# google-research/rigl

Hardware: NVIDIA H100
Metric: sparse_train_step_images_per_sec_resnet50_erk80 (higher is better)
Workload: dtype bf16

## Files before the change

rigl_b200/csrc/igemm_tc.cu:

```cuda
#include <cuda.h>
#include <cuda_bf16.h>

#include <stdio.h>
#include <stdlib.h>

#include <mutex>

#include "common.cuh"
#include "conv_common.cuh"
#include "tc_ptx.cuh"

namespace rigl {

using namespace ptx;

constexpr int kMaxTaps = 9;
constexpr int kBM = 128;
constexpr int kBK = 64;
constexpr int kThreads = 384;
constexpr int kConsumerWarp0 = 4;
constexpr int kConsumerWarps = 8;
constexpr int kConsumerThreads = 256;

struct TapInfo {
// ... 235 lines not shown
      }
    }
  } else if (warp >= kConsumerWarp0) {
    const int cw = warp - kConsumerWarp0;
    const int wg = cw >> 2;
    const int row = 64 * wg + 16 * (cw & 3) + (lane >> 2);
    const bool issuer = (cw == 0 && lane == 0);
    float acc[BN / 2];
    int stage = 0; uint32_t phase = 0;
    uint32_t slab_ctr = 0;
    uint32_t res_phase = 0;
    float* bn_row = (kEpi == kEpiPlain && p.bn_partial) ? p.bn_partial + (size_t)blockIdx.x * 2 * p.N : nullptr;
    if (bn_row) {
      for (int i = cw * 32 + lane; i < 2 * p.N; i += kConsumerThreads) bn_row[i] = 0.f;
      __threadfence_block();
      named_bar_sync(1, kConsumerThreads);
    }
    int tile_ctr = 0;
    for (int tile = first; tile < total; tile += step, ++tile_ctr) {
      const int n_tile = tile % p.n_tiles;
      const int m_tile = tile / p.n_tiles;
      uint32_t* live = live_cons[wg][tile_ctr & 1];
      if ((cw & 3) == 0) build_live_mask<kBN64>(p, n_tile, lane, live);
      named_bar_sync(3 + wg, 128);
      const bool masked = live_mask_used(p);
      zero_acc(acc);
      int prev = -1;
      const int nkb = p.ntaps * p.kblks;
      for (int j = 0; j < nkb; ++j) {
        if (masked && !((live[j >> 5] >> (j & 31)) & 1u)) continue;
        mbar_wait(full_bar(stage), phase);
        const uint32_t a_src = smem_base + stage * kStageBytes;
        const uint64_t da = make_smem_desc(a_src + (uint32_t)wg * 64u * 128u, 16, 1024);
        const uint64_t db = make_smem_desc(a_src + kABytes, 16, 1024);
        fence_regs(acc);
        wgmma_fence();
#pragma unroll
        for (int k = 0; k < kBK / 16; ++k)
          Wgmma<BN>::template ss<0, 0>(acc, da + 2 * k, db + 2 * k);
        wgmma_commit();
        wgmma_wait<1>();
        if (prev >= 0 && lane == 0) mbar_arrive(empty_bar(prev));
        prev = stage;
        if (++stage == STAGES) { stage = 0; phase ^= 1u; }
      }
      wgmma_wait<0>();
      fence_regs(acc);
      if (prev >= 0 && lane == 0) mbar_arrive(empty_bar(prev));

      const int tw = m_tile % p.tiles_w;
      const int th = (m_tile / p.tiles_w) % p.tiles_h;
      const int tn = m_tile / (p.tiles_w * p.tiles_h);
      bool ok[2]; long long o_pix[2];
#pragma unroll
      for (int h = 0; h < 2; ++h) {
        const int r = row + 8 * h;
        const int pw = tw * p.bw + r % p.bw;
        const int ph = th * p.bh + (r / p.bw) % p.bh;
        const int pn = tn * p.bn + r / (p.bw * p.bh);
        ok[h] = pw < p.GW && ph < p.GH && pn < p.NB;
        o_pix[h] = p.o_off + pn * p.o_sn + ph * p.o_sh + pw * p.o_sw;
      }
      if (kEpi != kEpiPlain || p.tma_store) {
#pragma unroll
        for (int s = 0; s < kBN64; ++s) {
          const int co0 = n_tile * BN + 64 * s;
          if (co0 >= p.N) break;
          const uint32_t slab = out_base + (uint32_t)(slab_ctr & 1) * kSlabBytes;
          if (issuer) tma_store_wait_read<1>();
          named_bar_sync(1, kConsumerThreads);
          if constexpr (kLoadsSlab) {
            if (kEpi == kEpiReluGate || ep.residual) {
              if (issuer) {
                mbar_arrive_expect_tx(res_bar, kSlabBytes);
                tma_load_4d(slab, rmap, res_bar, co0, tw * p.bw, th * p.bh, tn * p.bn);
              }
              mbar_wait(res_bar, res_phase);
              res_phase ^= 1u;
            }
          }
          if constexpr (kBnApply) {
            if (s == 0) stage_slab_bn<0>(acc, slab, row, ok[0], ok[1], lane, ep, co0, p.N);
            else stage_slab_bn<(kBN64 > 1 ? 1 : 0)>(acc, slab, row, ok[0], ok[1], lane, ep, co0, p.N);
          } else if constexpr (kEpi != kEpiPlain) {
            constexpr bool kGate = kEpi == kEpiReluGate;
            if (s == 0) stage_slab_relu<0, kGate>(acc, slab, row, ok[0], ok[1], lane);
            else stage_slab_relu<(kBN64 > 1 ? 1 : 0), kGate>(acc, slab, row, ok[0], ok[1], lane);
          } else {
            if (s == 0) stage_slab<0>(acc, slab, row, ok[0], ok[1], lane);
            else stage_slab<(kBN64 > 1 ? 1 : 0)>(acc, slab, row, ok[0], ok[1], lane);
          }
          fence_proxy_async_smem();
          named_bar_sync(1, kConsumerThreads);
          if (issuer) {
            tma_store_4d(&omap, slab, co0, tw * p.bw, th * p.bh, tn * p.bn);
            tma_store_commit();
          }
          if (bn_row && wg == 0) slab_bn_stats(slab, cw, lane, bn_row, co0, p.N);
          ++slab_ctr;
        }
      } else {
#pragma unroll
        for (int jc = 0; jc < BN / 8; ++jc) {
#pragma unroll
          for (int h = 0; h < 2; ++h) {
#pragma unroll
            for (int e = 0; e < 2; ++e) {
              const int co = n_tile * BN + 8 * jc + 2 * (lane & 3) + e;
              if (ok[h] && co < p.N) {
                float a = acc[4 * jc + 2 * h + e];
                if (p.bias) a += __ldg(p.bias + co);
                if (p.out_bf16) p.out_bf16[o_pix[h] + co] = __float2bfloat16(a);
                if (p.out_f32) p.out_f32[o_pix[h] + co] = a;
              }
            }
          }
        }
      }
    }
    if (p.tma_store && issuer) tma_store_wait_all();
  }
}

template <int BN, int STAGES>
__global__ void __launch_bounds__(kThreads, 1)
k_igemm_kmajor(const __grid_constant__ TMaps4 amaps, const __grid_constant__ CUtensorMap bmap,
               const __grid_constant__ CUtensorMap omap, const IgemmParams p) {
  kmajor_body<BN, STAGES, kEpiPlain>(amaps, bmap, omap, p, nullptr, BnEpilogue{});
}

template <int BN, int STAGES>
__global__ void __launch_bounds__(kThreads, 1)
k_igemm_kmajor_bn(const __grid_constant__ TMaps4 amaps, const __grid_constant__ CUtensorMap bmap,
                  const __grid_constant__ CUtensorMap omap, const IgemmParams p,
                  const __grid_constant__ CUtensorMap rmap, const BnEpilogue ep) {
  kmajor_body<BN, STAGES, kEpiBn>(amaps, bmap, omap, p, &rmap, ep);
}

template <int BN, int STAGES, bool kGate>
__global__ void __launch_bounds__(kThreads, 1)
k_igemm_kmajor_relu(const __grid_constant__ TMaps4 amaps, const __grid_constant__ CUtensorMap bmap,
                    const __grid_constant__ CUtensorMap omap, const IgemmParams p,
                    const __grid_constant__ CUtensorMap rmap) {
  kmajor_body<BN, STAGES, kGate ? kEpiReluGate : kEpiRelu>(amaps, bmap, omap, p, &rmap, BnEpilogue{});
}

struct WgradParams {
  int ntaps;
  TapInfo taps[kMaxTaps];
  int GW, GH, NB;
  int bw, bh, bn;
  int tiles_w, tiles_h, tiles_n;
  int pblocks, splits, pblocks_per_split;
  int ci, co;
  int m_tiles, n_tiles;
  float* out;
  long long split_stride;
};

template <int BN, int STAGES>
__global__ void __launch_bounds__(kThreads, 1)
k_igemm_wgrad(const __grid_constant__ TMaps4 xmaps, const __grid_constant__ CUtensorMap dymap,
              const WgradParams p) {
  extern __shared__ __align__(1024) uint8_t smem_raw[];
  constexpr uint32_t kABytes = kBM * kBK * 2;
  constexpr uint32_t kBBytes = BN * kBK * 2;
  constexpr uint32_t kStageBytes = kABytes + kBBytes;
  constexpr uint32_t kBox = 64 * 64 * 2;
  constexpr int kBBoxes = BN / 64;

  const uint32_t smem_base = (smem_u32(smem_raw) + 1023u) & ~1023u;
  const uint32_t bar_base = smem_base + STAGES * kStageBytes;
  auto full_bar = [&](int s) { return bar_base + 8u * s; };
  auto empty_bar = [&](int s) { return bar_base + 8u * (STAGES + s); };

  const int warp = threadIdx.x >> 5, lane = threadIdx.x & 31;
  if (threadIdx.x == 0) {
    for (int i = 0; i < 4; ++i) prefetch_tmap(&xmaps.a[i]);
    prefetch_tmap(&dymap);
    for (int s = 0; s < STAGES; ++s) { mbar_init(full_bar(s), 1); mbar_init(empty_bar(s), kConsumerWarps); }
    fence_barrier_init();
  }
  __syncthreads();

  const int mcount = p.ntaps * p.m_tiles;
  const int units_per_split = mcount * p.n_tiles;
  const int total_units = units_per_split * p.splits;
  const int first = blockIdx.x, step = gridDim.x;

  if (warp == 0) {
    int stage = 0; uint32_t phase = 0;
    for (int q = first; q < total_units; q += step) {
      const int split = q / units_per_split;
      const int r = q % units_per_split;
      const int n_tile = r % p.n_tiles;
      const int mi = r / p.n_tiles;
      const bool live = mi < mcount;
      const TapInfo tap = p.taps[live ? mi / p.m_tiles : 0];
      const int c_base = live ? (mi % p.m_tiles) * kBM : (1 << 28);
      const int pb0 = split * p.pblocks_per_split;
      const int pb1 = min(pb0 + p.pblocks_per_split, p.pblocks);
      int tw = pb0 % p.tiles_w, th = (pb0 / p.tiles_w) % p.tiles_h, tn = pb0 / (p.tiles_w * p.tiles_h);
      for (int pb = pb0; pb < pb1; ++pb) {
        mbar_wait(empty_bar(stage), phase ^ 1u);
        if (elect_one()) {
          const uint32_t a_dst = smem_base + stage * kStageBytes;
          const uint32_t b_dst = a_dst + kABytes;
          mbar_arrive_expect_tx(full_bar(stage), kStageBytes);
#pragma unroll
          for (int h = 0; h < kBM / 64; ++h)
            tma_load_4d(a_dst + h * kBox, &xmaps.a[tap.map_id], full_bar(stage), c_base + h * 64,
                        tw * p.bw + tap.dw, th * p.bh + tap.dh, tn * p.bn);
#pragma unroll
          for (int h = 0; h < kBBoxes; ++h)
            tma_load_4d(b_dst + h * kBox, &dymap, full_bar(stage), n_tile * BN + h * 64, tw * p.bw,
                        th * p.bh, tn * p.bn);
        }
        __syncwarp();
        if (++tw == p.tiles_w) { tw = 0; if (++th == p.tiles_h) { th = 0; ++tn; } }
        if (++stage == STAGES) { stage = 0; phase ^= 1u; }
      }
    }
  } else if (warp >= kConsumerWarp0) {
    const int cw = warp - kConsumerWarp0;
    const int wg = cw >> 2;
    const int row = 64 * wg + 16 * (cw & 3) + (lane >> 2);
    float acc[BN / 2];
    int stage = 0; uint32_t phase = 0;
    for (int q = first; q < total_units; q += step) {
      const int split = q / units_per_split;
      const int r = q % units_per_split;
      const int n_tile = r % p.n_tiles;
      const int mi = r / p.n_tiles;
      const bool live = mi < mcount;
      const int tap_idx = live ? mi / p.m_tiles : 0;
      const int pb0 = split * p.pblocks_per_split;
      const int pb1 = min(pb0 + p.pblocks_per_split, p.pblocks);
      zero_acc(acc);
      int prev = -1;
      for (int pb = pb0; pb < pb1; ++pb) {
        mbar_wait(full_bar(stage), phase);
        const uint32_t a_src = smem_base + stage * kStageBytes;
        const uint64_t da = make_smem_desc(a_src + (uint32_t)wg * kBox, kBox, 1024);
        const uint64_t db = make_smem_desc(a_src + kABytes, kBox, 1024);
        fence_regs(acc);
        wgmma_fence();
#pragma unroll
        for (int k = 0; k < kBK / 16; ++k)
          Wgmma<BN>::template ss<1, 1>(acc, da + 128 * k, db + 128 * k);
        wgmma_commit();
        wgmma_wait<1>();
        if (prev >= 0 && lane == 0) mbar_arrive(empty_bar(prev));
        prev = stage;
        if (++stage == STAGES) { stage = 0; phase ^= 1u; }
      }
      wgmma_wait<0>();
      fence_regs(acc);
      if (prev >= 0 && lane == 0) mbar_arrive(empty_bar(prev));

      const int m0 = live ? (mi % p.m_tiles) * kBM : p.ci;
      float* base = p.out + (long long)split * p.split_stride + (long long)p.taps[tap_idx].b_tap * p.ci * p.co;
#pragma unroll
      for (int h = 0; h < 2; ++h) {
        const int ci = m0 + row + 8 * h;
        if (ci >= p.ci) continue;
#pragma unroll
        for (int jc = 0; jc < BN / 8; ++jc) {
          const int co = n_tile * BN + 8 * jc + 2 * (lane & 3);
          if (co < p.co)
            *reinterpret_cast<float2*>(base + (long long)ci * p.co + co) =
                make_float2(acc[4 * jc + 2 * h], acc[4 * jc + 2 * h + 1]);
        }
      }
    }
  }
}

__global__ void k_splitk_reduce(const float* __restrict__ part, long long split_stride, int splits,
                                float* __restrict__ dw, long long n, float beta) {
  const long long i = ((long long)blockIdx.x * blockDim.x + threadIdx.x) * 4;
  if (i >= n) return;
  if (i + 3 < n) {
    float4 acc = beta != 0.f ? *reinterpret_cast<const float4*>(dw + i) : make_float4(0.f, 0.f, 0.f, 0.f);
    for (int s = 0; s < splits; ++s) {
      const float4 v = *reinterpret_cast<const float4*>(part + (long long)s * split_stride + i);
      acc.x += v.x; acc.y += v.y; acc.z += v.z; acc.w += v.w;
    }
    *reinterpret_cast<float4*>(dw + i) = acc;
  } else {
    for (long long j = i; j < n; ++j) {
      float a = beta != 0.f ? dw[j] : 0.f;
      for (int s = 0; s < splits; ++s) a += part[(long long)s * split_stride + j];
      dw[j] = a;
    }
  }
}

typedef CUresult (*EncodeTiledFn)(CUtensorMap*, CUtensorMapDataType, cuuint32_t, void*, const cuuint64_t*,
                                  const cuuint64_t*, const cuuint32_t*, const cuuint32_t*, CUtensorMapInterleave,
                                  CUtensorMapSwizzle, CUtensorMapL2promotion, CUtensorMapFloatOOBfill);

static EncodeTiledFn g_encode = nullptr;
static bool g_bn_stats_always = false;
static bool g_halo = true;
static int g_num_sms = 0;
static std::once_flag g_once;
static int g_init_status = RIGL_OK;

static void init_driver() {
  void* fn = nullptr;
  cudaDriverEntryPointQueryResult qres;
  cudaError_t e = cudaGetDriverEntryPoint("cuTensorMapEncodeTiled", &fn, cudaEnableDefault, &qres);
  if (e != cudaSuccess || fn == nullptr || qres != cudaDriverEntryPointSuccess) {
    set_error("cuTensorMapEncodeTiled not available from the driver (%s)", cudaGetErrorString(e));
    g_init_status = RIGL_ERR_DRIVER;
    return;
  }
  g_encode = reinterpret_cast<EncodeTiledFn>(fn);
  if (const char* e = getenv("RIGL_HALO3X3")) g_halo = !(e[0] == '0');
  int dev = 0;
  cudaGetDevice(&dev);
  cudaDeviceGetAttribute(&g_num_sms, cudaDevAttrMultiProcessorCount, dev);
  if (g_num_sms <= 0) g_num_sms = kNumSmsHint;
}

static int ensure_driver() {
  static thread_local bool ctx_ready = false;
  if (!ctx_ready) {
    cudaFree(0);
    ctx_ready = true;
  }
  std::call_once(g_once, init_driver);
  return g_init_status;
}

static int make_tmap_swz(CUtensorMap* out, const void* base, int rank, const uint64_t* dims,
                         const uint64_t* strides_bytes , const uint32_t* box, CUtensorMapSwizzle swz) {
  cuuint32_t estr[5] = {1, 1, 1, 1, 1};
  cuuint64_t gdim[5], gstr[4];
  cuuint32_t bx[5];
  for (int i = 0; i < rank; ++i) { gdim[i] = dims[i]; bx[i] = box[i]; }
  for (int i = 0; i + 1 < rank; ++i) gstr[i] = strides_bytes[i];
  CUresult r = g_encode(out, CU_TENSOR_MAP_DATA_TYPE_BFLOAT16, (cuuint32_t)rank, const_cast<void*>(base), gdim,
                        gstr, bx, estr, CU_TENSOR_MAP_INTERLEAVE_NONE, swz,
                        CU_TENSOR_MAP_L2_PROMOTION_L2_128B, CU_TENSOR_MAP_FLOAT_OOB_FILL_NONE);
  if (r != CUDA_SUCCESS) {
    set_error("cuTensorMapEncodeTiled failed (%d): rank %d dims [%llu,%llu,%llu,%llu] box [%u,%u,%u,%u]", (int)r,
              rank, (unsigned long long)dims[0], (unsigned long long)(rank > 1 ? dims[1] : 0),
              (unsigned long long)(rank > 2 ? dims[2] : 0), (unsigned long long)(rank > 3 ? dims[3] : 0), box[0],
              rank > 1 ? box[1] : 0, rank > 2 ? box[2] : 0, rank > 3 ? box[3] : 0);
    return RIGL_ERR_DRIVER;
  }
  return RIGL_OK;
}
static int make_tmap(CUtensorMap* out, const void* base, int rank, const uint64_t* dims,
                     const uint64_t* strides_bytes , const uint32_t* box) {
  return make_tmap_swz(out, base, rank, dims, strides_bytes, box, CU_TENSOR_MAP_SWIZZLE_128B);
}

static int make_act_map(CUtensorMap* out, const void* base, int nb, int h, int w, int c, int pitch, int s, int rh,
                        int rw, const uint32_t box[4]) {
  const uint64_t hr = (h - rh + s - 1) / s, wr = (w - rw + s - 1) / s;
  const uint64_t dims[4] = {(uint64_t)c, wr, hr, (uint64_t)nb};
  const uint64_t strides[3] = {(uint64_t)s * pitch * 2, (uint64_t)s * w * pitch * 2, (uint64_t)h * w * pitch * 2};
  const uint8_t* p = static_cast<const uint8_t*>(base) + ((size_t)rh * w + rw) * pitch * 2;
  return make_tmap(out, p, 4, dims, strides, box);
}

static void choose_box(int gw, int gh, int nb, int total, int* bw, int* bh, int* bn) {
  long long best = -1;
  for (int w = 1; w <= total; w *= 2)
    for (int h = 1; w * h <= total; h *= 2) {
      const int n = total / (w * h);
      const long long padded = (long long)((gw + w - 1) / w * w) * ((gh + h - 1) / h * h) * ((nb + n - 1) / n * n);
      const long long score = padded * 1024 - w * 16 - h;
      if (best < 0 || score < best) { best = score; *bw = w; *bh = h; *bn = n; }
    }
}

static inline int floordiv(int a, int b) { return (a >= 0) ? a / b : -((-a + b - 1) / b); }
static inline int posmod(int a, int b) { return ((a % b) + b) % b; }

template <typename P>
static void set_pixel_tiling(P& p, int gw, int gh, int nb, int box_pixels) {
  p.GW = gw; p.GH = gh; p.NB = nb;
  choose_box(gw, gh, nb, box_pixels, &p.bw, &p.bh, &p.bn);
  p.tiles_w = (gw + p.bw - 1) / p.bw; p.tiles_h = (gh + p.bh - 1) / p.bh; p.tiles_n = (nb + p.bn - 1) / p.bn;
}

template <typename P>
static int set_conv_taps(P& p, TMaps4* maps, const ConvGeom& g, const void* x, const uint32_t box[4]) {
  bool made[4] = {false, false, false, false};
  p.ntaps = 0;
  for (int kh = 0; kh < g.ksize; ++kh)
    for (int kw = 0; kw < g.ksize; ++kw) {
      const int rh = posmod(kh - g.pad, g.stride), rw = posmod(kw - g.pad, g.stride);
      const int id = rh * g.stride + rw;
      if (!made[id]) {
        const int rc = make_act_map(&maps->a[id], x, g.batch, g.in_h, g.in_w, g.cin, g.x_pitch, g.stride, rh, rw, box);
        if (rc != RIGL_OK) return rc;
        made[id] = true;
      }
      TapInfo& t = p.taps[p.ntaps++];
      t.map_id = (int8_t)id; t.dh = (int8_t)floordiv(kh - g.pad, g.stride); t.dw = (int8_t)floordiv(kw - g.pad, g.stride);
      t.b_tap = kh * g.ksize + kw;
    }
  for (int i = 0; i < 4; ++i) if (!made[i]) maps->a[i] = maps->a[p.taps[0].map_id];
  return RIGL_OK;
}

int tc_max_ctas() {
  ensure_driver();
  return g_num_sms > 0 ? g_num_sms : kNumSmsHint;
}

bool tc_supported(const ConvGeom& g, int which) {
  if (g.x_pitch % 8 || g.cout % 8) return false;
  if (which == 1 && g.cin % 8) return false;
  if (g.stride != 1 && g.stride != 2) return false;
  if (g.ksize * g.ksize > kMaxTaps) return false;
  (void)which;
  return true;
}

// ... 98 lines not shown
  int rc = ensure_driver();
  if (rc != RIGL_OK) return rc;
  const PackedLayout L = packed_layout(g.taps(), g.cin, g.cout);
  const uint8_t* pk = static_cast<const uint8_t*>(packed);
  {
    HaloParams hp = {};
    if (y != nullptr && y_f32 == nullptr && bias == nullptr && halo_fprop_ok(g, &hp)) {
      if (relu)
        return halo_launch_kmajor(hp, x, g.cin, g.x_pitch, pk + L.off_fprop, L.cin_pad, g.cout, y, g.cout, false, s,
                                  true);
      if (bn_apply != nullptr) {
        set_error("fused BN apply: layer runs on the halo kernels");
        return RIGL_ERR_UNSUPPORTED;
      }
      if (bn_partial != nullptr) {
        set_error("fused BN statistics: layer runs on the halo kernels");
        return RIGL_ERR_UNSUPPORTED;
      }
      return halo_launch_kmajor(hp, x, g.cin, g.x_pitch, pk + L.off_fprop, L.cin_pad, g.cout, y, g.cout, false, s);
    }
  }
  if (bn_partial != nullptr && !g_bn_stats_always) {
    const int K = g.taps() * g.cin;
    if (!(K >= 512 || (K >= 256 && g.cout <= 128))) {
      set_error("fused BN statistics: not profitable for this shape (K = %d, cout = %d)", K, g.cout);
      return RIGL_ERR_UNSUPPORTED;
    }
  }
  IgemmParams p = {};
  set_pixel_tiling(p, g.out_w, g.out_h, g.batch, 128);
  p.kblks = (g.cin + kBK - 1) / kBK;
  p.N = g.cout;
  p.out_bf16 = static_cast<__nv_bfloat16*>(y); p.out_f32 = y_f32; p.bias = bias;
  p.o_off = 0; p.o_sw = g.cout; p.o_sh = (long long)g.out_w * g.cout; p.o_sn = (long long)g.out_h * g.out_w * g.cout;
  p.nnz = reinterpret_cast<const uint32_t*>(pk + L.off_nnz);
  p.nnz_tap_stride = L.n_tiles * L.k_tiles; p.nnz_n_stride = L.k_tiles; p.nnz_k_stride = 1;
  p.bn_partial = bn_partial;
  TMaps4 amaps;
  const uint32_t abox[4] = {(uint32_t)kBK, (uint32_t)p.bw, (uint32_t)p.bh, (uint32_t)p.bn};
  rc = set_conv_taps(p, &amaps, g, x, abox);
  if (rc != RIGL_OK) return rc;
  const int bn_tile = pick_bn(g.cout);
  CUtensorMap bmap;
  const uint64_t bdims[3] = {(uint64_t)L.cin_pad, (uint64_t)g.cout, (uint64_t)g.taps()};
  const uint64_t bstr[2] = {(uint64_t)L.cin_pad * 2, (uint64_t)g.cout * L.cin_pad * 2};
  const uint32_t bbox[3] = {(uint32_t)kBK, (uint32_t)bn_tile, 1};
  rc = make_tmap(&bmap, pk + L.off_fprop, 3, bdims, bstr, bbox);
  if (rc != RIGL_OK) return rc;
  CUtensorMap omap = bmap;
  p.tma_store = (y != nullptr && y_f32 == nullptr && bias == nullptr) ? 1 : 0;
  if (p.tma_store) {
    rc = make_act_map(&omap, y, g.batch, g.out_h, g.out_w, g.cout, g.cout, 1, 0, 0, abox);
    if (rc != RIGL_OK) return rc;
  }
  if (bn_partial) {
    p.bn_partial = bn_partial;
    p.n_tiles = (g.cout + bn_tile - 1) / bn_tile;
    if (bn_rows) *bn_rows = kmajor_grid(p);
  }
  if (bn_apply) {
    CUtensorMap rmap = omap;
    if (bn_apply->residual) {
      rc = make_act_map(&rmap, bn_apply->residual, g.batch, g.out_h, g.out_w, g.cout, g.cout, 1, 0, 0, abox);
      if (rc != RIGL_OK) return rc;
    }
    const BnEpilogue ep = {bn_apply->scale, bn_apply->shift, bn_apply->relu ? 1 : 0, bn_apply->residual ? 1 : 0};
    return dispatch_kmajor(g.cout, amaps, bmap, omap, p, bn_tile, s, &rmap, &ep);
  }
  if (relu) return dispatch_kmajor(g.cout, amaps, bmap, omap, p, bn_tile, s, nullptr, nullptr, kReluFprop);
  return dispatch_kmajor(g.cout, amaps, bmap, omap, p, bn_tile, s);
}

int tc_dgrad(const ConvGeom& g, const void* dy, const void* packed, void* dx, void* ws, size_t ws_bytes,
             cudaStream_t s, const void* gate) {
  (void)ws; (void)ws_bytes;
  int rc = ensure_driver();
  if (rc != RIGL_OK) return rc;
  const PackedLayout L = packed_layout(g.taps(), g.cin, g.cout);
  const uint8_t* pk = static_cast<const uint8_t*>(packed);
  const int st = g.stride;
  {
    HaloParams hp = {};
    if (halo_dgrad_ok(g, &hp)) {
      if (gate != nullptr) {
        set_error("gated dgrad: layer runs on the halo kernels");
        return RIGL_ERR_UNSUPPORTED;
      }
      return halo_launch_kmajor(hp, dy, g.cout, g.cout, pk + L.off_dgrad, L.cout_pad, g.cin, dx, g.x_pitch, true, s);
    }
  }
  if (gate != nullptr && st != 1) {
    set_error("gated dgrad: only the single-launch stride-1 dgrad has the gate");
    return RIGL_ERR_UNSUPPORTED;
  }
  bool need_zero = false;
  for (int ph = 0; ph < st && !need_zero; ++ph)
    for (int pw = 0; pw < st; ++pw) {
      int n = 0;
      for (int kh = 0; kh < g.ksize; ++kh)
        for (int kw = 0; kw < g.ksize; ++kw)
          if (posmod(ph + g.pad - kh, st) == 0 && posmod(pw + g.pad - kw, st) == 0) ++n;
      if (n == 0) need_zero = true;
    }
  if (need_zero) RIGL_CUDA(cudaMemsetAsync(dx, 0, (size_t)g.in_pixels() * g.x_pitch * 2, s));
  for (int ph = 0; ph < st; ++ph)
    for (int pw = 0; pw < st; ++pw) {
      IgemmParams p = {};
      const int gh = (g.in_h - ph + st - 1) / st, gw = (g.in_w - pw + st - 1) / st;
      if (gh <= 0 || gw <= 0) continue;
      p.ntaps = 0;
      for (int kh = 0; kh < g.ksize; ++kh)
        for (int kw = 0; kw < g.ksize; ++kw)
          if (posmod(ph + g.pad - kh, st) == 0 && posmod(pw + g.pad - kw, st) == 0) {
            TapInfo& t = p.taps[p.ntaps++];
            t.map_id = 0; t.dh = (int8_t)((ph + g.pad - kh) / st); t.dw = (int8_t)((pw + g.pad - kw) / st);
            t.b_tap = kh * g.ksize + kw;
          }
      if (p.ntaps == 0) continue;
      set_pixel_tiling(p, gw, gh, g.batch, 128);
      p.kblks = (g.cout + kBK - 1) / kBK;
      p.N = g.cin;
      p.nnz = reinterpret_cast<const uint32_t*>(pk + L.off_nnz);
      p.nnz_tap_stride = L.n_tiles * L.k_tiles; p.nnz_n_stride = 1; p.nnz_k_stride = L.k_tiles;
      TMaps4 amaps;
      const uint32_t abox[4] = {(uint32_t)kBK, (uint32_t)p.bw, (uint32_t)p.bh, (uint32_t)p.bn};
      rc = make_act_map(&amaps.a[0], dy, g.batch, g.out_h, g.out_w, g.cout, g.cout, 1, 0, 0, abox);
      if (rc != RIGL_OK) return rc;
      for (int i = 1; i < 4; ++i) amaps.a[i] = amaps.a[0];
      const int bn_tile = pick_bn(g.cin);
      CUtensorMap bmap;
      const uint64_t bdims[3] = {(uint64_t)L.cout_pad, (uint64_t)g.cin, (uint64_t)g.taps()};
      const uint64_t bstr[2] = {(uint64_t)L.cout_pad * 2, (uint64_t)g.cin * L.cout_pad * 2};
      const uint32_t bbox[3] = {(uint32_t)kBK, (uint32_t)bn_tile, 1};
      rc = make_tmap(&bmap, pk + L.off_dgrad, 3, bdims, bstr, bbox);
      if (rc != RIGL_OK) return rc;
      CUtensorMap omap;
      rc = make_act_map(&omap, dx, g.batch, g.in_h, g.in_w, g.cin, g.x_pitch, st, ph, pw, abox);
      if (rc != RIGL_OK) return rc;
      p.tma_store = 1;
      if (gate != nullptr) {
        CUtensorMap xmap;
        rc = make_act_map(&xmap, gate, g.batch, g.in_h, g.in_w, g.cin, g.x_pitch, st, ph, pw, abox);
        if (rc != RIGL_OK) return rc;
        rc = dispatch_kmajor(g.cin, amaps, bmap, omap, p, bn_tile, s, &xmap, nullptr, kReluGateDgrad);
        if (rc != RIGL_OK) return rc;
        continue;
      }
      rc = dispatch_kmajor(g.cin, amaps, bmap, omap, p, bn_tile, s);
      if (rc != RIGL_OK) return rc;
    }
  return RIGL_OK;
}

template <int BN, int STAGES>
static int launch_wgrad(const TMaps4& xmaps, const CUtensorMap& dymap, const WgradParams& p, cudaStream_t s) {
  constexpr size_t smem = (size_t)STAGES * (kBM * kBK * 2 + BN * kBK * 2) + 1024 + 256;
  static_assert(smem <= 227 * 1024, "wgrad kernel exceeds the shared memory of an SM");
  static bool configured = false;
  if (!configured) {
    RIGL_CUDA(cudaFuncSetAttribute(k_igemm_wgrad<BN, STAGES>, cudaFuncAttributeMaxDynamicSharedMemorySize, (int)smem));
    configured = true;
  }
  const int units = p.ntaps * p.m_tiles * p.n_tiles * p.splits;
  const int grid = units < g_num_sms ? units : g_num_sms;
  k_igemm_wgrad<BN, STAGES><<<grid, kThreads, smem, s>>>(xmaps, dymap, p);
  RIGL_LAUNCH_CHECK("k_igemm_wgrad");
  return RIGL_OK;
}

int tc_wgrad(const ConvGeom& g, const void* x, const void* dy, float* dw, float beta, void* ws, size_t ws_bytes,
             cudaStream_t s) {
  int rc = ensure_driver();
  if (rc != RIGL_OK) return rc;
  {
    HaloParams hp = {};
    if (halo_wgrad_ok(g, &hp)) {
      const size_t need = halo_wgrad_ws_elems(g, hp) * sizeof(float);
      float* wsf = reinterpret_cast<float*>((reinterpret_cast<uintptr_t>(ws) + 255) & ~(uintptr_t)255);
      if (ws == nullptr || ws_bytes < need + 256) {
        set_error("rigl_conv2d_wgrad_dense: workspace %zu < required %zu", ws_bytes, need + 256);
        return RIGL_ERR_WORKSPACE;
      }
      rc = halo_launch_wgrad(hp, g, x, dy, wsf, s);
      if (rc != RIGL_OK) return rc;
      const long long n_w9 = (long long)9 * g.cin * g.cout;
      const long long threads = (n_w9 + 3) / 4;
      k_splitk_reduce<<<(unsigned)((threads + 255) / 256), 256, 0, s>>>(wsf, n_w9, halo_wgrad_grid(hp), dw, n_w9, beta);
      RIGL_LAUNCH_CHECK("k_splitk_reduce");
      return RIGL_OK;
    }
  }
  WgradParams p = {};
  set_pixel_tiling(p, g.out_w, g.out_h, g.batch, 64);
  p.pblocks = p.tiles_w * p.tiles_h * p.tiles_n;
  const int bn_tile = wgrad_bn_tile(g);
  const size_t elems = wgrad_ws_elems(g, &p.splits, &p.pblocks_per_split, p.bw, p.bh, p.bn, bn_tile);
  p.ci = g.cin; p.co = g.cout;
  p.m_tiles = (g.cin + kBM - 1) / kBM; p.n_tiles = (g.cout + bn_tile - 1) / bn_tile;
  const long long n_w = (long long)g.taps() * g.cin * g.cout;
  const bool direct = (p.splits == 1 && beta == 0.f);
  if (!direct) {
    const size_t need = elems * sizeof(float);
    if (ws == nullptr || ws_bytes < need + 256) {
      set_error("rigl_conv2d_wgrad_dense: workspace %zu < required %zu", ws_bytes, need + 256);
      return RIGL_ERR_WORKSPACE;
    }
    p.out = reinterpret_cast<float*>((reinterpret_cast<uintptr_t>(ws) + 255) & ~(uintptr_t)255);
    p.split_stride = n_w;
  } else {
    p.out = dw; p.split_stride = 0;
  }
  TMaps4 xmaps;
  const uint32_t box[4] = {64, (uint32_t)p.bw, (uint32_t)p.bh, (uint32_t)p.bn};
  rc = set_conv_taps(p, &xmaps, g, x, box);
  if (rc != RIGL_OK) return rc;
  CUtensorMap dymap;
  rc = make_act_map(&dymap, dy, g.batch, g.out_h, g.out_w, g.cout, g.cout, 1, 0, 0, box);
  if (rc != RIGL_OK) return rc;
  rc = (bn_tile == 128) ? launch_wgrad<128, 6>(xmaps, dymap, p, s) : launch_wgrad<64, 8>(xmaps, dymap, p, s);
  if (rc != RIGL_OK) return rc;
  if (!direct) {
    const long long threads = (n_w + 3) / 4;
    k_splitk_reduce<<<(unsigned)((threads + 255) / 256), 256, 0, s>>>(p.out, p.split_stride, p.splits, dw, n_w, beta);
    RIGL_LAUNCH_CHECK("k_splitk_reduce");
  }
  return RIGL_OK;
}

}
```

rigl_b200/csrc/tc_ptx.cuh:

```cuda
#pragma once
#include <cuda.h>
#include <cuda_runtime.h>
#include <stdint.h>

namespace rigl {
namespace ptx {

__device__ __forceinline__ uint32_t smem_u32(const void* p) {
  return static_cast<uint32_t>(__cvta_generic_to_shared(p));
}

__device__ __forceinline__ bool elect_one() {
  uint32_t pred;
  asm volatile(
      "{\n"
      ".reg .pred p;\n"
      "elect.sync _|p, 0xffffffff;\n"
      "selp.u32 %0, 1, 0, p;\n"
      "}\n"
      : "=r"(pred));
  return pred != 0;
}

__device__ __forceinline__ void mbar_init(uint32_t bar, uint32_t count) {
  asm volatile("mbarrier.init.shared::cta.b64 [%0], %1;" ::"r"(bar), "r"(count) : "memory");
}
__device__ __forceinline__ void fence_barrier_init() {
  asm volatile("fence.mbarrier_init.release.cluster;" ::: "memory");
}
__device__ __forceinline__ void mbar_arrive_expect_tx(uint32_t bar, uint32_t bytes) {
  asm volatile("mbarrier.arrive.expect_tx.shared::cta.b64 _, [%0], %1;" ::"r"(bar), "r"(bytes) : "memory");
}
__device__ __forceinline__ void mbar_arrive(uint32_t bar) {
  asm volatile("mbarrier.arrive.shared::cta.b64 _, [%0];" ::"r"(bar) : "memory");
}
__device__ __forceinline__ void mbar_wait(uint32_t bar, uint32_t parity) {
  uint32_t done;
  uint32_t spins = 0;
  long long t0 = 0;
  do {
    asm volatile(
        "{\n"
        ".reg .pred p;\n"
        "mbarrier.try_wait.parity.shared::cta.b64 p, [%1], %2;\n"
        "selp.u32 %0, 1, 0, p;\n"
        "}\n"
        : "=r"(done)
        : "r"(bar), "r"(parity)
        : "memory");
    if (!done && (++spins & 0xFFFu) == 0) {
      const long long now = clock64();
      if (t0 == 0) t0 = now;
      else if (now - t0 > 8000000000ll) __trap();
    }
  } while (!done);
}

__device__ __forceinline__ void prefetch_tmap(const CUtensorMap* m) {
  asm volatile("prefetch.tensormap [%0];" ::"l"(reinterpret_cast<uint64_t>(m)) : "memory");
}
__device__ __forceinline__ void tma_load_4d(uint32_t dst, const CUtensorMap* m, uint32_t bar, int c0, int c1,
                                            int c2, int c3) {
  asm volatile(
      "cp.async.bulk.tensor.4d.shared::cluster.global.mbarrier::complete_tx::bytes [%0], [%1, {%3, %4, %5, %6}], [%2];"
      ::"r"(dst), "l"(reinterpret_cast<uint64_t>(m)), "r"(bar), "r"(c0), "r"(c1), "r"(c2), "r"(c3)
      : "memory");
}
__device__ __forceinline__ void tma_load_3d(uint32_t dst, const CUtensorMap* m, uint32_t bar, int c0, int c1,
                                            int c2) {
  asm volatile(
      "cp.async.bulk.tensor.3d.shared::cluster.global.mbarrier::complete_tx::bytes [%0], [%1, {%3, %4, %5}], [%2];"
      ::"r"(dst), "l"(reinterpret_cast<uint64_t>(m)), "r"(bar), "r"(c0), "r"(c1), "r"(c2)
      : "memory");
}

__device__ __forceinline__ void tma_store_4d(const CUtensorMap* m, uint32_t src, int c0, int c1, int c2, int c3) {
  asm volatile("cp.async.bulk.tensor.4d.global.shared::cta.bulk_group [%0, {%2, %3, %4, %5}], [%1];" ::"l"(
                   reinterpret_cast<uint64_t>(m)),
               "r"(src), "r"(c0), "r"(c1), "r"(c2), "r"(c3)
               : "memory");
}
__device__ __forceinline__ void tma_store_commit() { asm volatile("cp.async.bulk.commit_group;" ::: "memory"); }
template <int N>
__device__ __forceinline__ void tma_store_wait_read() {
  asm volatile("cp.async.bulk.wait_group.read %0;" ::"n"(N) : "memory");
}
__device__ __forceinline__ void tma_store_wait_all() { asm volatile("cp.async.bulk.wait_group 0;" ::: "memory"); }
__device__ __forceinline__ void fence_proxy_async_smem() { asm volatile("fence.proxy.async.shared::cta;" ::: "memory"); }
__device__ __forceinline__ void named_bar_sync(int id, int nthreads) {
  asm volatile("bar.sync %0, %1;" ::"r"(id), "r"(nthreads) : "memory");
}

__device__ __forceinline__ void wgmma_fence() { asm volatile("wgmma.fence.sync.aligned;" ::: "memory"); }
__device__ __forceinline__ void wgmma_commit() { asm volatile("wgmma.commit_group.sync.aligned;" ::: "memory"); }
template <int N>
__device__ __forceinline__ void wgmma_wait() {
  asm volatile("wgmma.wait_group.sync.aligned %0;" ::"n"(N) : "memory");
}
template <int R>
__device__ __forceinline__ void fence_regs(float (&d)[R]) {
#pragma unroll
  for (int i = 0; i < R; ++i) asm volatile("" : "+f"(d[i])::"memory");
}

constexpr uint32_t kSwz128 = 1, kSwz32 = 3;
__device__ __forceinline__ uint64_t make_smem_desc(uint32_t saddr, uint32_t lbo_bytes, uint32_t sbo_bytes,
                                                   uint32_t swz = kSwz128) {
  uint64_t d = 0;
  d |= (uint64_t)((saddr >> 4) & 0x3FFFu);
  d |= (uint64_t)((lbo_bytes >> 4) & 0x3FFFu) << 16;
  d |= (uint64_t)((sbo_bytes >> 4) & 0x3FFFu) << 32;
  d |= (uint64_t)swz << 62;
  return d;
}

__device__ __forceinline__ void ldmatrix_x4(uint32_t (&r)[4], uint32_t addr) {
  asm volatile("ldmatrix.sync.aligned.m8n8.x4.shared.b16 {%0, %1, %2, %3}, [%4];"
               : "=r"(r[0]), "=r"(r[1]), "=r"(r[2]), "=r"(r[3]) : "r"(addr) : "memory");
}
__device__ __forceinline__ void ldmatrix_x4_trans(uint32_t (&r)[4], uint32_t addr) {
  asm volatile("ldmatrix.sync.aligned.m8n8.x4.trans.shared.b16 {%0, %1, %2, %3}, [%4];"
               : "=r"(r[0]), "=r"(r[1]), "=r"(r[2]), "=r"(r[3]) : "r"(addr) : "memory");
}
__device__ __forceinline__ uint32_t swz128(uint32_t addr) { return addr ^ (((addr >> 7) & 7u) << 4); }
__device__ __forceinline__ uint32_t swz32(uint32_t addr) { return addr ^ (((addr >> 7) & 1u) << 4); }

template <int N> struct Wgmma;
template <> struct Wgmma<64> {
  template <int TA, int TB>
  static __device__ __forceinline__ void ss(float (&d)[32], uint64_t da, uint64_t db) {
    asm volatile(
        "{\n.reg .pred p;\nsetp.ne.b32 p, 1, 0;\nwgmma.mma_async.sync.aligned.m64n64k16.f32.bf16.bf16 "
        "{%0, %1, %2, %3, %4, %5, %6, %7, %8, %9, %10, %11, %12, %13, %14, %15, %16, %17, %18, %19, %20, %21, %22, %23, %24, %25, %26, %27, %28, %29, %30, %31}, %32, %33, p, 1, 1, %34, %35;\n}\n"
        : "+f"(d[0]), "+f"(d[1]), "+f"(d[2]), "+f"(d[3]), "+f"(d[4]), "+f"(d[5]), "+f"(d[6]), "+f"(d[7]), "+f"(d[8]), "+f"(d[9]), "+f"(d[10]), "+f"(d[11]), "+f"(d[12]), "+f"(d[13]), "+f"(d[14]), "+f"(d[15]), "+f"(d[16]), "+f"(d[17]), "+f"(d[18]), "+f"(d[19]), "+f"(d[20]), "+f"(d[21]), "+f"(d[22]), "+f"(d[23]), "+f"(d[24]), "+f"(d[25]), "+f"(d[26]), "+f"(d[27]), "+f"(d[28]), "+f"(d[29]), "+f"(d[30]), "+f"(d[31])
        : "l"(da), "l"(db), "n"(TA), "n"(TB));
  }
  template <int TB>
  static __device__ __forceinline__ void rs(float (&d)[32], const uint32_t (&a)[4], uint64_t db) {
    asm volatile(
        "{\n.reg .pred p;\nsetp.ne.b32 p, 1, 0;\nwgmma.mma_async.sync.aligned.m64n64k16.f32.bf16.bf16 "
        "{%0, %1, %2, %3, %4, %5, %6, %7, %8, %9, %10, %11, %12, %13, %14, %15, %16, %17, %18, %19, %20, %21, %22, %23, %24, %25, %26, %27, %28, %29, %30, %31}, {%32, %33, %34, %35}, %36, p, 1, 1, %37;\n}\n"
        : "+f"(d[0]), "+f"(d[1]), "+f"(d[2]), "+f"(d[3]), "+f"(d[4]), "+f"(d[5]), "+f"(d[6]), "+f"(d[7]), "+f"(d[8]), "+f"(d[9]), "+f"(d[10]), "+f"(d[11]), "+f"(d[12]), "+f"(d[13]), "+f"(d[14]), "+f"(d[15]), "+f"(d[16]), "+f"(d[17]), "+f"(d[18]), "+f"(d[19]), "+f"(d[20]), "+f"(d[21]), "+f"(d[22]), "+f"(d[23]), "+f"(d[24]), "+f"(d[25]), "+f"(d[26]), "+f"(d[27]), "+f"(d[28]), "+f"(d[29]), "+f"(d[30]), "+f"(d[31])
        : "r"(a[0]), "r"(a[1]), "r"(a[2]), "r"(a[3]), "l"(db), "n"(TB));
  }
};
template <> struct Wgmma<128> {
  template <int TA, int TB>
  static __device__ __forceinline__ void ss(float (&d)[64], uint64_t da, uint64_t db) {
    asm volatile(
        "{\n.reg .pred p;\nsetp.ne.b32 p, 1, 0;\nwgmma.mma_async.sync.aligned.m64n128k16.f32.bf16.bf16 "
        "{%0, %1, %2, %3, %4, %5, %6, %7, %8, %9, %10, %11, %12, %13, %14, %15, %16, %17, %18, %19, %20, %21, %22, %23, %24, %25, %26, %27, %28, %29, %30, %31, %32, %33, %34, %35, %36, %37, %38, %39, %40, %41, %42, %43, %44, %45, %46, %47, %48, %49, %50, %51, %52, %53, %54, %55, %56, %57, %58, %59, %60, %61, %62, %63}, %64, %65, p, 1, 1, %66, %67;\n}\n"
        : "+f"(d[0]), "+f"(d[1]), "+f"(d[2]), "+f"(d[3]), "+f"(d[4]), "+f"(d[5]), "+f"(d[6]), "+f"(d[7]), "+f"(d[8]), "+f"(d[9]), "+f"(d[10]), "+f"(d[11]), "+f"(d[12]), "+f"(d[13]), "+f"(d[14]), "+f"(d[15]), "+f"(d[16]), "+f"(d[17]), "+f"(d[18]), "+f"(d[19]), "+f"(d[20]), "+f"(d[21]), "+f"(d[22]), "+f"(d[23]), "+f"(d[24]), "+f"(d[25]), "+f"(d[26]), "+f"(d[27]), "+f"(d[28]), "+f"(d[29]), "+f"(d[30]), "+f"(d[31]), "+f"(d[32]), "+f"(d[33]), "+f"(d[34]), "+f"(d[35]), "+f"(d[36]), "+f"(d[37]), "+f"(d[38]), "+f"(d[39]), "+f"(d[40]), "+f"(d[41]), "+f"(d[42]), "+f"(d[43]), "+f"(d[44]), "+f"(d[45]), "+f"(d[46]), "+f"(d[47]), "+f"(d[48]), "+f"(d[49]), "+f"(d[50]), "+f"(d[51]), "+f"(d[52]), "+f"(d[53]), "+f"(d[54]), "+f"(d[55]), "+f"(d[56]), "+f"(d[57]), "+f"(d[58]), "+f"(d[59]), "+f"(d[60]), "+f"(d[61]), "+f"(d[62]), "+f"(d[63])
        : "l"(da), "l"(db), "n"(TA), "n"(TB));
  }
  template <int TB>
  static __device__ __forceinline__ void rs(float (&d)[64], const uint32_t (&a)[4], uint64_t db) {
    asm volatile(
        "{\n.reg .pred p;\nsetp.ne.b32 p, 1, 0;\nwgmma.mma_async.sync.aligned.m64n128k16.f32.bf16.bf16 "
        "{%0, %1, %2, %3, %4, %5, %6, %7, %8, %9, %10, %11, %12, %13, %14, %15, %16, %17, %18, %19, %20, %21, %22, %23, %24, %25, %26, %27, %28, %29, %30, %31, %32, %33, %34, %35, %36, %37, %38, %39, %40, %41, %42, %43, %44, %45, %46, %47, %48, %49, %50, %51, %52, %53, %54, %55, %56, %57, %58, %59, %60, %61, %62, %63}, {%64, %65, %66, %67}, %68, p, 1, 1, %69;\n}\n"
        : "+f"(d[0]), "+f"(d[1]), "+f"(d[2]), "+f"(d[3]), "+f"(d[4]), "+f"(d[5]), "+f"(d[6]), "+f"(d[7]), "+f"(d[8]), "+f"(d[9]), "+f"(d[10]), "+f"(d[11]), "+f"(d[12]), "+f"(d[13]), "+f"(d[14]), "+f"(d[15]), "+f"(d[16]), "+f"(d[17]), "+f"(d[18]), "+f"(d[19]), "+f"(d[20]), "+f"(d[21]), "+f"(d[22]), "+f"(d[23]), "+f"(d[24]), "+f"(d[25]), "+f"(d[26]), "+f"(d[27]), "+f"(d[28]), "+f"(d[29]), "+f"(d[30]), "+f"(d[31]), "+f"(d[32]), "+f"(d[33]), "+f"(d[34]), "+f"(d[35]), "+f"(d[36]), "+f"(d[37]), "+f"(d[38]), "+f"(d[39]), "+f"(d[40]), "+f"(d[41]), "+f"(d[42]), "+f"(d[43]), "+f"(d[44]), "+f"(d[45]), "+f"(d[46]), "+f"(d[47]), "+f"(d[48]), "+f"(d[49]), "+f"(d[50]), "+f"(d[51]), "+f"(d[52]), "+f"(d[53]), "+f"(d[54]), "+f"(d[55]), "+f"(d[56]), "+f"(d[57]), "+f"(d[58]), "+f"(d[59]), "+f"(d[60]), "+f"(d[61]), "+f"(d[62]), "+f"(d[63])
        : "r"(a[0]), "r"(a[1]), "r"(a[2]), "r"(a[3]), "l"(db), "n"(TB));
  }
};

}
}
```

Baseline: 6567.

## Split wgrad tail-wave tiles into N-halves and fuse beta accumulation

When the wgrad work units leave a partial last wave across SMs, the tail units are split into two 64-wide N halves and run in a second launch, so more SMs share the tail. The direct (no split-K) path now also handles beta by reading and adding the existing gradient in the epilogue, which avoids the workspace and the separate reduce kernel when splits==1. The cost is an extra kernel launch, narrower m64n64 tensor-core ops for the tail, and a read-modify-write in the epilogue.

After: 6612, median of 6. Within noise of the previous version (+0.7%).

```diff
diff --git a/rigl_b200/csrc/igemm_tc.cu b/rigl_b200/csrc/igemm_tc.cu
--- a/rigl_b200/csrc/igemm_tc.cu
+++ b/rigl_b200/csrc/igemm_tc.cu
@@ -411,13 +411,22 @@
   int bw, bh, bn;
   int tiles_w, tiles_h, tiles_n;
   int pblocks, splits, pblocks_per_split;
+  int full, halves;
   int ci, co;
   int m_tiles, n_tiles;
   float* out;
   long long split_stride;
+  float beta;
 };
 
-template <int BN, int STAGES>
+template <bool kHalf>
+__device__ __forceinline__ int wgrad_item(const WgradParams& p, int q, int* half) {
+  if (!kHalf) { *half = -1; return q; }
+  *half = q & 1;
+  return p.full + (q >> 1);
+}
+
+template <int BN, int STAGES, bool kHalf>
 __global__ void __launch_bounds__(kThreads, 1)
 k_igemm_wgrad(const __grid_constant__ TMaps4 xmaps, const __grid_constant__ CUtensorMap dymap,
               const WgradParams p) {
@@ -444,12 +453,15 @@
 
   const int mcount = p.ntaps * p.m_tiles;
   const int units_per_split = mcount * p.n_tiles;
-  const int total_units = units_per_split * p.splits;
+  static_assert(!kHalf || BN == 128, "only 128-wide N tiles have halves");
+  const int total_items = kHalf ? p.halves : p.full;
   const int first = blockIdx.x, step = gridDim.x;
 
   if (warp == 0) {
     int stage = 0; uint32_t phase = 0;
-    for (int q = first; q < total_units; q += step) {
+    for (int item = first; item < total_items; item += step) {
+      int half;
+      const int q = wgrad_item<kHalf>(p, item, &half);
       const int split = q / units_per_split;
       const int r = q % units_per_split;
       const int n_tile = r % p.n_tiles;
@@ -465,15 +477,19 @@
         if (elect_one()) {
           const uint32_t a_dst = smem_base + stage * kStageBytes;
           const uint32_t b_dst = a_dst + kABytes;
-          mbar_arrive_expect_tx(full_bar(stage), kStageBytes);
+          mbar_arrive_expect_tx(full_bar(stage), kHalf ? kABytes + kBox : kStageBytes);
 #pragma unroll
           for (int h = 0; h < kBM / 64; ++h)
             tma_load_4d(a_dst + h * kBox, &xmaps.a[tap.map_id], full_bar(stage), c_base + h * 64,
                         tw * p.bw + tap.dw, th * p.bh + tap.dh, tn * p.bn);
-#pragma unroll
-          for (int h = 0; h < kBBoxes; ++h)
-            tma_load_4d(b_dst + h * kBox, &dymap, full_bar(stage), n_tile * BN + h * 64, tw * p.bw,
-                        th * p.bh, tn * p.bn);
+          if constexpr (!kHalf) {
+#pragma unroll
+            for (int h = 0; h < kBBoxes; ++h)
+              tma_load_4d(b_dst + h * kBox, &dymap, full_bar(stage), n_tile * BN + h * 64, tw * p.bw,
+                          th * p.bh, tn * p.bn);
+          } else {
+            tma_load_4d(b_dst, &dymap, full_bar(stage), n_tile * BN + half * 64, tw * p.bw, th * p.bh, tn * p.bn);
+          }
         }
         __syncwarp();
         if (++tw == p.tiles_w) { tw = 0; if (++th == p.tiles_h) { th = 0; ++tn; } }
@@ -486,7 +502,9 @@
     const int row = 64 * wg + 16 * (cw & 3) + (lane >> 2);
     float acc[BN / 2];
     int stage = 0; uint32_t phase = 0;
-    for (int q = first; q < total_units; q += step) {
+    for (int item = first; item < total_items; item += step) {
+      int half;
+      const int q = wgrad_item<kHalf>(p, item, &half);
       const int split = q / units_per_split;
       const int r = q % units_per_split;
       const int n_tile = r % p.n_tiles;
@@ -504,9 +522,15 @@
         const uint64_t db = make_smem_desc(a_src + kABytes, kBox, 1024);
         fence_regs(acc);
         wgmma_fence();
-#pragma unroll
-        for (int k = 0; k < kBK / 16; ++k)
-          Wgmma<BN>::template ss<1, 1>(acc, da + 128 * k, db + 128 * k);
+        if constexpr (!kHalf) {
+#pragma unroll
+          for (int k = 0; k < kBK / 16; ++k)
+            Wgmma<BN>::template ss<1, 1>(acc, da + 128 * k, db + 128 * k);
+        } else {
+#pragma unroll
+          for (int k = 0; k < kBK / 16; ++k)
+            Wgmma<BN>::template ss_lo<1, 1>(acc, da + 128 * k, db + 128 * k);
+        }
         wgmma_commit();
         wgmma_wait<1>();
         if (prev >= 0 && lane == 0) mbar_arrive(empty_bar(prev));
@@ -518,6 +542,9 @@
       if (prev >= 0 && lane == 0) mbar_arrive(empty_bar(prev));
 
       const int m0 = live ? (mi % p.m_tiles) * kBM : p.ci;
+      const bool add_old = p.splits == 1 && p.beta != 0.f;
+      const int co0 = n_tile * BN + (half > 0 ? 64 : 0);
+      constexpr int jcs = kHalf ? 8 : BN / 8;
       float* base = p.out + (long long)split * p.split_stride + (long long)p.taps[tap_idx].b_tap * p.ci * p.co;
 #pragma unroll
       for (int h = 0; h < 2; ++h) {
@@ -525,10 +552,13 @@
         if (ci >= p.ci) continue;
 #pragma unroll
         for (int jc = 0; jc < BN / 8; ++jc) {
-          const int co = n_tile * BN + 8 * jc + 2 * (lane & 3);
-          if (co < p.co)
-            *reinterpret_cast<float2*>(base + (long long)ci * p.co + co) =
-                make_float2(acc[4 * jc + 2 * h], acc[4 * jc + 2 * h + 1]);
+          const int co = co0 + 8 * jc + 2 * (lane & 3);
+          if (jc < jcs && co < p.co) {
+            float2* dst = reinterpret_cast<float2*>(base + (long long)ci * p.co + co);
+            float2 v = make_float2(acc[4 * jc + 2 * h], acc[4 * jc + 2 * h + 1]);
+            if (add_old) { const float2 o = *dst; v.x = o.x + v.x; v.y = o.y + v.y; }
+            *dst = v;
+          }
         }
       }
     }
@@ -933,18 +963,19 @@
   return RIGL_OK;
 }
 
-template <int BN, int STAGES>
+template <int BN, int STAGES, bool kHalf>
 static int launch_wgrad(const TMaps4& xmaps, const CUtensorMap& dymap, const WgradParams& p, cudaStream_t s) {
   constexpr size_t smem = (size_t)STAGES * (kBM * kBK * 2 + BN * kBK * 2) + 1024 + 256;
   static_assert(smem <= 227 * 1024, "wgrad kernel exceeds the shared memory of an SM");
   static bool configured = false;
   if (!configured) {
-    RIGL_CUDA(cudaFuncSetAttribute(k_igemm_wgrad<BN, STAGES>, cudaFuncAttributeMaxDynamicSharedMemorySize, (int)smem));
+    RIGL_CUDA(cudaFuncSetAttribute(k_igemm_wgrad<BN, STAGES, kHalf>, cudaFuncAttributeMaxDynamicSharedMemorySize,
+                                   (int)smem));
     configured = true;
   }
-  const int units = p.ntaps * p.m_tiles * p.n_tiles * p.splits;
-  const int grid = units < g_num_sms ? units : g_num_sms;
-  k_igemm_wgrad<BN, STAGES><<<grid, kThreads, smem, s>>>(xmaps, dymap, p);
+  const int items = kHalf ? p.halves : p.full;
+  const int grid = items < g_num_sms ? items : g_num_sms;
+  k_igemm_wgrad<BN, STAGES, kHalf><<<grid, kThreads, smem, s>>>(xmaps, dymap, p);
   RIGL_LAUNCH_CHECK("k_igemm_wgrad");
   return RIGL_OK;
 }
@@ -979,7 +1010,13 @@
   p.ci = g.cin; p.co = g.cout;
   p.m_tiles = (g.cin + kBM - 1) / kBM; p.n_tiles = (g.cout + bn_tile - 1) / bn_tile;
   const long long n_w = (long long)g.taps() * g.cin * g.cout;
-  const bool direct = (p.splits == 1 && beta == 0.f);
+  const int units = g.taps() * p.m_tiles * p.n_tiles * p.splits;
+  const int tail = units % g_num_sms;
+  const bool halve = bn_tile == 128 && units > g_num_sms && tail > 0 && 2 * tail <= g_num_sms;
+  p.full = halve ? units - tail : units;
+  p.halves = halve ? 2 * tail : 0;
+  p.beta = beta;
+  const bool direct = p.splits == 1;
   if (!direct) {
     const size_t need = elems * sizeof(float);
     if (ws == nullptr || ws_bytes < need + 256) {
@@ -998,8 +1035,12 @@
   CUtensorMap dymap;
   rc = make_act_map(&dymap, dy, g.batch, g.out_h, g.out_w, g.cout, g.cout, 1, 0, 0, box);
   if (rc != RIGL_OK) return rc;
-  rc = (bn_tile == 128) ? launch_wgrad<128, 6>(xmaps, dymap, p, s) : launch_wgrad<64, 8>(xmaps, dymap, p, s);
+  rc = (bn_tile == 128) ? launch_wgrad<128, 6, false>(xmaps, dymap, p, s) : launch_wgrad<64, 8, false>(xmaps, dymap, p, s);
   if (rc != RIGL_OK) return rc;
+  if (p.halves > 0) {
+    rc = launch_wgrad<128, 6, true>(xmaps, dymap, p, s);
+    if (rc != RIGL_OK) return rc;
+  }
   if (!direct) {
     const long long threads = (n_w + 3) / 4;
     k_splitk_reduce<<<(unsigned)((threads + 255) / 256), 256, 0, s>>>(p.out, p.split_stride, p.splits, dw, n_w, beta);
diff --git a/rigl_b200/csrc/tc_ptx.cuh b/rigl_b200/csrc/tc_ptx.cuh
--- a/rigl_b200/csrc/tc_ptx.cuh
+++ b/rigl_b200/csrc/tc_ptx.cuh
@@ -146,6 +146,14 @@
 };
 template <> struct Wgmma<128> {
   template <int TA, int TB>
+  static __device__ __forceinline__ void ss_lo(float (&d)[64], uint64_t da, uint64_t db) {
+    asm volatile(
+        "{\n.reg .pred p;\nsetp.ne.b32 p, 1, 0;\nwgmma.mma_async.sync.aligned.m64n64k16.f32.bf16.bf16 "
+        "{%0, %1, %2, %3, %4, %5, %6, %7, %8, %9, %10, %11, %12, %13, %14, %15, %16, %17, %18, %19, %20, %21, %22, %23, %24, %25, %26, %27, %28, %29, %30, %31}, %32, %33, p, 1, 1, %34, %35;\n}\n"
+        : "+f"(d[0]), "+f"(d[1]), "+f"(d[2]), "+f"(d[3]), "+f"(d[4]), "+f"(d[5]), "+f"(d[6]), "+f"(d[7]), "+f"(d[8]), "+f"(d[9]), "+f"(d[10]), "+f"(d[11]), "+f"(d[12]), "+f"(d[13]), "+f"(d[14]), "+f"(d[15]), "+f"(d[16]), "+f"(d[17]), "+f"(d[18]), "+f"(d[19]), "+f"(d[20]), "+f"(d[21]), "+f"(d[22]), "+f"(d[23]), "+f"(d[24]), "+f"(d[25]), "+f"(d[26]), "+f"(d[27]), "+f"(d[28]), "+f"(d[29]), "+f"(d[30]), "+f"(d[31])
+        : "l"(da), "l"(db), "n"(TA), "n"(TB));
+  }
+  template <int TA, int TB>
   static __device__ __forceinline__ void ss(float (&d)[64], uint64_t da, uint64_t db) {
     asm volatile(
         "{\n.reg .pred p;\nsetp.ne.b32 p, 1, 0;\nwgmma.mma_async.sync.aligned.m64n128k16.f32.bf16.bf16 "
```
